# alexandre01/deepsvg

Measured on AMD Instinct MI355X. Metric: SVG icons/sec (train step) hierarchical_ordered d=256, higher is better.
Workload: dtype bf16; 1 GPU; hierarchical_ordered (Hierarchical, use_vae=False) G=8 S=30 d_model=256 ff=512 H=8 L=4x4; full train step = forward + SVGLoss + backward + grad-clip 1.0 + AdamW; dropout 0.1; global_batch=512, batch_per_gpu=512, parallelism=dp1, hip_graph=True, encoder_layout=packed (valid tokens only, exact)

## Files before the change

### deepsvg_amd/csrc/layernorm.hip

```cpp
#include "dsvg_common.h"
#include "../../include/dsvg.h"

constexpr int LN_MAXV_MAX = 4;
constexpr int LN_MAX_BLOCKS = 1024;

template <typename T, int LN_MAXV>
__global__ __launch_bounds__(256) void ln_fwd_kernel(const T* __restrict__ x, const float* __restrict__ gamma,
                                                     const float* __restrict__ beta, T* __restrict__ y,
                                                     float* __restrict__ mean, float* __restrict__ rstd,
                                                     long long rows, int d, float eps) {
    const int lane = threadIdx.x & 63;
    const int wave = threadIdx.x >> 6;
    const int nv = d / 256 + ((d % 256) ? 1 : 0);
    float4 g4[LN_MAXV], b4[LN_MAXV];
#pragma unroll
    for (int i = 0; i < LN_MAXV; ++i) {
        const int c = min(i * 256 + lane * 4, d - 4);
        g4[i] = *reinterpret_cast<const float4*>(gamma + c);
        b4[i] = *reinterpret_cast<const float4*>(beta + c);
    }
    for (long long row = (long long)blockIdx.x * 4 + wave; row < rows; row += (long long)gridDim.x * 4) {
        const T* xr = x + row * d;
        float v[LN_MAXV][4];
        float s = 0.f;
#pragma unroll
        for (int i = 0; i < LN_MAXV; ++i) {
            const int c = i * 256 + lane * 4;
            if (i < nv && c < d) {
                Elem<T>::ld4(xr + c, v[i]);
                s += v[i][0] + v[i][1] + v[i][2] + v[i][3];
            } else {
                v[i][0] = v[i][1] = v[i][2] = v[i][3] = 0.f;
            }
        }
        const float mu = wave_sum(s) / (float)d;
        float s2 = 0.f;
#pragma unroll
        for (int i = 0; i < LN_MAXV; ++i) {
            const int c = i * 256 + lane * 4;
            if (i < nv && c < d) {
#pragma unroll
                for (int e = 0; e < 4; ++e) { const float t = v[i][e] - mu; s2 += t * t; }
            }
        }
        const float var = wave_sum(s2) / (float)d;
        const float rs = rsqrtf(var + eps);
        if (lane == 0) { mean[row] = mu; rstd[row] = rs; }
        T* yr = y + row * d;
#pragma unroll
        for (int i = 0; i < LN_MAXV; ++i) {
            const int c = i * 256 + lane * 4;
            if (i < nv && c < d) {
                const float4 g = g4[i];
                const float4 b = b4[i];
                float o[4];
                o[0] = (v[i][0] - mu) * rs * g.x + b.x;
                o[1] = (v[i][1] - mu) * rs * g.y + b.y;
                o[2] = (v[i][2] - mu) * rs * g.z + b.z;
                o[3] = (v[i][3] - mu) * rs * g.w + b.w;
                Elem<T>::st4(yr + c, o);
            }
        }
    }
}

template <typename T, int LN_MAXV>
__global__ __launch_bounds__(256) void ln_bwd_kernel(const T* dy, const T* __restrict__ x,
                                                     const float* __restrict__ mean, const float* __restrict__ rstd,
                                                     const float* __restrict__ gamma, const T* res,
                                                     T* dx, float* __restrict__ part,
                                                     long long rows, int d, T* dxm, float drop_p,
                                                     const uint64_t* __restrict__ seed, uint32_t site) {
    const DropCtx dmc = drop_make(dxm ? drop_p : 0.f, seed, site);
    extern __shared__ float red_raw[];
    const int nvec = d / 4 + 1;
    auto red = [&](int w, int k, int vec, int e) -> float& { return red_raw[((w * 2 + k) * nvec + vec) * 4 + e]; };
    const int lane = threadIdx.x & 63;
    const int wave = threadIdx.x >> 6;
    const int nv = d / 256 + ((d % 256) ? 1 : 0);
    float ag[LN_MAXV][4], ab[LN_MAXV][4];
#pragma unroll
    for (int i = 0; i < LN_MAXV; ++i)
#pragma unroll
        for (int e = 0; e < 4; ++e) { ag[i][e] = 0.f; ab[i][e] = 0.f; }

    float4 g4[LN_MAXV];
#pragma unroll
    for (int i = 0; i < LN_MAXV; ++i) g4[i] = *reinterpret_cast<const float4*>(gamma + min(i * 256 + lane * 4, d - 4));
    for (long long row = (long long)blockIdx.x * 4 + wave; row < rows; row += (long long)gridDim.x * 4) {
        const float mu = mean[row], rs = rstd[row];
        float xh[LN_MAXV][4], gd[LN_MAXV][4], rv[LN_MAXV][4];
        float c1 = 0.f, c2 = 0.f;
#pragma unroll
        for (int i = 0; i < LN_MAXV; ++i) {
            const int c = i * 256 + lane * 4;
            if (i < nv && c < d) {
                float xv[4], dv[4];
                Elem<T>::ld4(x + row * d + c, xv);
                Elem<T>::ld4(dy + row * d + c, dv);
                if (res) Elem<T>::ld4(res + row * d + c, rv[i]);
                const float4 g = g4[i];
                const float gg[4] = {g.x, g.y, g.z, g.w};
#pragma unroll
                for (int e = 0; e < 4; ++e) {
                    xh[i][e] = (xv[e] - mu) * rs;
                    gd[i][e] = gg[e] * dv[e];
                    c1 += gd[i][e];
                    c2 += gd[i][e] * xh[i][e];
                    ag[i][e] += dv[e] * xh[i][e];
                    ab[i][e] += dv[e];
                }
            } else {
#pragma unroll
                for (int e = 0; e < 4; ++e) { xh[i][e] = 0.f; gd[i][e] = 0.f; }
// ... 83 lines not shown
    else if (dtype == DSVG_BF16) { if (d <= 256) DSVG_LNF(bf16_t, 1); else if (d <= 512) DSVG_LNF(bf16_t, 2); else DSVG_LNF(bf16_t, 4); }
    else { dsvg_set_error("layernorm_fwd: bad dtype %d", dtype); return -1; }
#undef DSVG_LNF
    DSVG_LAUNCH_CHECK("layernorm_fwd");
    return 0;
}

extern "C" int64_t dsvg_layernorm_bwd_workspace_bytes(int64_t rows, int32_t d) {
    return (int64_t)ln_grid(rows) * 2 * d * (int64_t)sizeof(float);
}

static int ln_bwd_launch(int32_t dtype, const void* dy, const void* x, const float* mean, const float* rstd,
                         const float* gamma, const void* res, void* dx, float* dgamma, float* dbeta,
                         int32_t accumulate, int64_t rows, int32_t d, float* workspace,
                         int64_t workspace_bytes, void* dx_masked, float drop_p, uint32_t drop_site, const void* seed,
                         void* stream);

extern "C" int dsvg_layernorm_bwd(int32_t dtype, const void* dy, const void* x, const float* mean, const float* rstd,
                                  const float* gamma, const void* res, void* dx, float* dgamma, float* dbeta,
                                  int32_t accumulate, int64_t rows, int32_t d, float* workspace,
                                  int64_t workspace_bytes, void* stream) {
    return ln_bwd_launch(dtype, dy, x, mean, rstd, gamma, res, dx, dgamma, dbeta, accumulate, rows, d, workspace,
                         workspace_bytes, nullptr, 0.f, 0u, nullptr, stream);
}

extern "C" int dsvg_layernorm_bwd_masked(int32_t dtype, const void* dy, const void* x, const float* mean, const float* rstd,
                                         const float* gamma, const void* res, void* dx, float* dgamma, float* dbeta,
                                         int32_t accumulate, int64_t rows, int32_t d, float* workspace,
                                         int64_t workspace_bytes, void* dx_masked, float drop_p, uint32_t drop_site,
                                         const void* seed, void* stream) {
    DSVG_CHECK_ARG(dx_masked && dx_masked != dx, "layernorm_bwd_masked: needs a second output buffer");
    DSVG_CHECK_ARG(!(drop_p > 0.f) || seed, "layernorm_bwd_masked: dropout needs a seed");
    return ln_bwd_launch(dtype, dy, x, mean, rstd, gamma, res, dx, dgamma, dbeta, accumulate, rows, d, workspace,
                         workspace_bytes, dx_masked, drop_p, drop_site, seed, stream);
}

static int ln_bwd_launch(int32_t dtype, const void* dy, const void* x, const float* mean, const float* rstd,
                         const float* gamma, const void* res, void* dx, float* dgamma, float* dbeta,
                         int32_t accumulate, int64_t rows, int32_t d, float* workspace,
                         int64_t workspace_bytes, void* dx_masked, float drop_p, uint32_t drop_site, const void* seed,
                         void* stream) {
    DSVG_CHECK_ARG(dy && x && mean && rstd && gamma && dx && dgamma && dbeta, "layernorm_bwd: null pointer");
    DSVG_CHECK_ARG(rows > 0 && d > 0 && (d % 4) == 0 && d <= 1024, "layernorm_bwd: bad shape");
    DSVG_CHECK_ARG(workspace && workspace_bytes >= dsvg_layernorm_bwd_workspace_bytes(rows, d),
                   "layernorm_bwd: workspace too small");
    hipStream_t st = (hipStream_t)stream;
    const int nb = ln_grid(rows);
    const size_t lds = (size_t)4 * 2 * (d / 4 + 1) * 4 * sizeof(float);
#define DSVG_LNB(TT, NV) hipLaunchKernelGGL((ln_bwd_kernel<TT, NV>), dim3(nb), dim3(256), lds, st, (const TT*)dy, \
                                            (const TT*)x, mean, rstd, gamma, (const TT*)res, (TT*)dx, workspace,  \
                                            (long long)rows, d, (TT*)dx_masked, drop_p, (const uint64_t*)seed, drop_site)
    if (dtype == DSVG_F32) { if (d <= 256) DSVG_LNB(float, 1); else if (d <= 512) DSVG_LNB(float, 2); else DSVG_LNB(float, 4); }
    else if (dtype == DSVG_BF16) { if (d <= 256) DSVG_LNB(bf16_t, 1); else if (d <= 512) DSVG_LNB(bf16_t, 2); else DSVG_LNB(bf16_t, 4); }
    else { dsvg_set_error("layernorm_bwd: bad dtype %d", dtype); return -1; }
#undef DSVG_LNB
    DSVG_LAUNCH_CHECK("layernorm_bwd");
    if (dbeta == dgamma + d)
        return dsvg_reduce_partials_strided(workspace, nb, 2 * (int64_t)d, 2 * (int64_t)d, dgamma, accumulate, st);
    int rc = 0;
    rc = dsvg_reduce_partials_strided(workspace, nb, 2 * (int64_t)d, d, dgamma, accumulate, st);
    if (rc) return rc;
    rc = dsvg_reduce_partials_strided(workspace + d, nb, 2 * (int64_t)d, d, dbeta, accumulate, st);
    return rc;
}
```

### deepsvg_amd/functional.py

```python
import math
import contextlib
import functools
import os

import torch

from . import ops

FFN_MIN_ROWS = int(os.environ.get("DSVG_FFN_MIN_ROWS", "16384"))
ATTN_MIN_ROWS = int(os.environ.get("DSVG_ATTN_MIN_ROWS", "16384"))
FFN_GATE_DW2 = os.environ.get("DSVG_FFN_GATE_DW2", "1") != "0"

LN_BWD_MASKED = os.environ.get("DSVG_LN_BWD_MASKED", "1") != "0"
DEFER_MORE = os.environ.get("DSVG_DEFER_MORE", "1") != "0"
HEAD_KPAD = os.environ.get("DSVG_HEAD_KPAD", "1") != "0"
GS_STACK = os.environ.get("DSVG_GS_STACK", "1") != "0"
_ATTN_VALU = os.environ.get("DSVG_ATTN_VALU") is not None
_ATTN_MFMA_MIN_S = int(os.environ.get("DSVG_ATTN_MFMA_MIN_S", "2"))
ATTN_BWD_DX = os.environ.get("DSVG_ATTN_BWD_DX", "0") != "0"
ATTN_BWD_DX_MIN_ROWS = int(os.environ.get("DSVG_ATTN_BWD_DX_MIN_ROWS", "8192"))
GS_REMAINDER = int(os.environ.get("DSVG_GS_REMAINDER", "512"))
SEQ_ROUND = 2048
HEAD_FUSED = os.environ.get("DSVG_HEAD_FUSED", "0") != "0"

# ... 271 lines not shown
            mk = (rt.p(ctx.mask_below[0]), ctx.mask_below[1], rt.seed)
        with rt.deferring():
            if live is None:
                out = ops.layernorm_bwd(dy, x, mean, rstd, gamma.detach(),
                                        dgamma=rt.grad_out(gamma), dbeta=rt.grad_out(beta), masked=mk)
                dx, dg, db = out[:3]
            else:
                R = live[1]
                dx = torch.empty_like(x)
                out = ops.layernorm_bwd(dy[:R], x[:R], mean[:R], rstd[:R], gamma.detach(), dx=dx[:R],
                                        dgamma=rt.grad_out(gamma), dbeta=rt.grad_out(beta), masked=mk)
                dg, db = out[1:3]
        if mk is not None:
            _hand_masked(rt, dx, out[3], mk[0], mk[1])
        return None, dx, dg, db, None, None, None


class AddPosFn(torch.autograd.Function):

    @staticmethod
    def forward(ctx, rt, x, pos_weight, n_seq, S, drop_rate, site, live=None):
        p = rt.p(drop_rate)
        y = ops.add_pos_fwd(x, pos_weight.detach(), n_seq, S, rt.dtype, p, site, rt.seed)
        ctx.rt, ctx.n_seq, ctx.S, ctx.p, ctx.site = rt, n_seq, S, p, site
        ctx.has_x = x is not None
        ctx.live = _live_rows(live, n_seq * S)
        assert ctx.live is None or x is None, "live-prefix backward is only wired for the constant embedding"
        ctx.save_for_backward(pos_weight)
        return y

# ... 766 lines not shown
```

### deepsvg_amd/lib.py

```python
import ctypes as C
import os

_HERE = os.path.dirname(os.path.abspath(__file__))
LIB_PATH = os.path.join(_HERE, "_lib", "libdsvg_hip.so")

DSVG_F32 = 0
DSVG_BF16 = 1
ABI_VERSION = 11

c_i32, c_i64, c_u32, c_f32 = C.c_int32, C.c_int64, C.c_uint32, C.c_float
vp = C.c_void_p


class GemmDesc(C.Structure):
    _fields_ = [
        ("dtype", c_i32), ("M", c_i32), ("N", c_i32), ("K", c_i32),
        ("A", vp), ("lda", c_i64), ("a_kc", c_i32),
        ("B", vp), ("ldb", c_i64), ("b_kc", c_i32),
        ("C", vp), ("ldc", c_i64), ("c_f32", c_i32),
        ("bias", vp),
        ("res", vp), ("ldres", c_i64), ("res_pre", c_i32),
        ("act", c_i32),
        ("gate", vp), ("ldgate", c_i64), ("gate_scale", c_f32),
        ("drop_p", c_f32), ("drop_site", c_u32),
# ... 23 lines not shown
    "dsvg_version": (c_i32, []),
    "dsvg_gemm": (c_i32, [C.POINTER(GemmDesc), vp]),
    "dsvg_gemm_workspace_bytes": (c_i64, [c_i32, c_i32, c_i32]),
    "dsvg_reduce_partials": (c_i32, [vp, c_i64, c_i64, vp, c_i32, vp]),
    "dsvg_defer_scope": (c_i32, [c_i32, vp]),
    "dsvg_flush_deferred": (c_i32, [vp]),
    "dsvg_defer_zero": (c_i32, [vp, c_i64, vp]),
    "dsvg_gemm_group_scope": (c_i32, [c_i32, vp]),
    "dsvg_colsum": (c_i32, [c_i32, vp, c_i64, c_i64, c_i32, vp, c_i32, c_f32, c_u32, vp, vp, c_i64, vp]),
    "dsvg_colsum_workspace_bytes": (c_i64, [c_i64, c_i32]),
    "dsvg_layernorm_fwd": (c_i32, [c_i32, vp, vp, vp, vp, vp, vp, c_i64, c_i32, c_f32, vp]),
    "dsvg_layernorm_bwd": (c_i32, [c_i32, vp, vp, vp, vp, vp, vp, vp, vp, vp, c_i32, c_i64, c_i32, vp, c_i64, vp]),
    "dsvg_layernorm_bwd_workspace_bytes": (c_i64, [c_i64, c_i32]),
    "dsvg_layernorm_bwd_masked": (c_i32, [c_i32, vp, vp, vp, vp, vp, vp, vp, vp, vp, c_i32, c_i64, c_i32, vp, c_i64, vp, c_f32,
                                          c_u32, vp, vp]),
    "dsvg_attention_fwd": (c_i32, [c_i32, vp, vp, vp, c_i64, vp, vp, c_i64, c_i32, c_i32, c_f32, c_f32, c_u32, vp, vp]),
    "dsvg_attention_bwd": (c_i32, [c_i32, vp, vp, vp, c_i64, vp, vp, vp, c_i64, c_i32, c_i32, c_f32, c_f32, c_u32, vp, vp]),
    "dsvg_attention_tiles": (c_i32, [vp, c_i64, c_i32, vp, vp, vp]),
    "dsvg_pack_tokens": (c_i32, [vp, vp, vp, c_i64, c_i32, c_i32, vp, vp, vp, vp, vp]),
    "dsvg_visible_first": (c_i32, [vp, c_i64, vp, vp, vp, vp]),
    "dsvg_head_pack_elems": (c_i64, [c_i32]),
    "dsvg_head_pack": (c_i32, [vp, c_i32, vp, vp]),
    "dsvg_head_argmax": (c_i32, [vp, vp, vp, c_i64, c_i32, c_i32, vp, vp]),
    "dsvg_head_sample": (c_i32, [vp, vp, vp, c_i64, c_i32, c_i32, c_f32, vp, c_u32, vp, vp]),
    "dsvg_head_lse_workspace_bytes": (c_i64, [c_i64]),
    "dsvg_head_lse": (c_i32, [vp, vp, vp, c_i64, c_i32, c_i32, vp, vp, vp, vp, vp, vp, c_i64, vp]),
    "dsvg_head_dlogits": (c_i32, [vp, vp, vp, c_i64, c_i32, c_i32, vp, vp, vp, vp, vp, vp, c_f32, vp, c_i64, vp]),
    "dsvg_attention_bwd_outproj": (c_i32, [vp, vp, vp, c_i64, vp, vp, vp, vp, c_i64, c_i32, c_f32, c_f32, c_u32, vp, vp]),
    "dsvg_attn_pack_bwd_elems": (c_i64, [c_i32]),
    "dsvg_attn_pack_bwd": (c_i32, [vp, vp, c_i32, vp, vp]),
# ... 122 lines not shown
```

### deepsvg_amd/model.py

```python
import math
import os

import torch
import torch.nn as nn

from . import ops
from . import functional as Fn
from .svgtensor import CMD_ARGS_MASK, EOS_ID, M_ID, SOS_ID

PACK_ONE_LAUNCH = os.environ.get("DSVG_PACK_ONE", "1") != "0"
PE_DROPOUT = 0.1


class ModelOutput(dict):
    _PENDING = object()

    def __init__(self, *a, **k):
        super().__init__(*a, **k)
        self._thunks = {}

    def set_lazy(self, key, fn):
        self._thunks[key] = fn
        dict.__setitem__(self, key, ModelOutput._PENDING)

# ... 563 lines not shown
    def seed_tensor(self, device):
        if self._seed is None or self._seed.device != device:
            self._seed = torch.tensor([torch.initial_seed() & 0x7FFFFFFFFFFFFFFF], dtype=torch.int64, device=device)
        return self._seed

    def _runtime(self, device):
        training = self.training
        seed = self.seed_tensor(device) if training else None
        self._store.ensure(device, self.compute_dtype, advance=(None, seed) if training and self._own_seed else None)
        self._rt = Fn.Runtime(self.compute_dtype, seed, self._store, training,
                              defer=self._defer_wgrad and (not ops.PROFILE_ON or ops.PROFILE_KEEP_DEFER))
        self._rt.path_stage = self.cfg.encode_stages == 2 or self.cfg.decode_stages == 2
        return self._rt

    def _run_stack(self, rt, stack, x, key_mask, z, n_seq, S, site, seq_off=None, live=None, tiles=None, l=None,
                   causal=False):
        cfg = self.cfg
        gl = None
        if z is not None and all(hasattr(L, "linear_global") for L in stack.layers) and self.hoist_global:
            wb = [t for L in stack.layers for t in (L.linear_global.weight, L.linear_global.bias)]
            gl = Fn.GlobalCondFn.apply(rt, z, *wb)
        n = len(stack.layers)
        all_g = all(hasattr(L, "linear_global") for L in stack.layers)
        if (n > 0 and not causal and seq_off is None and live is None and tiles is None and l is None
                and (z is None or (gl is not None and all_g))
                and Fn.gs_stack_eligible(rt, x, key_mask, n_seq, S, cfg.n_heads, n, [L.self_attn.in_proj_weight for L in stack.layers])):
            ts = []
            for i, L in enumerate(stack.layers):
                ts += [L.norm1.weight, L.norm1.bias, L.self_attn.in_proj_weight, L.self_attn.in_proj_bias,
                       L.self_attn.out_proj.weight, L.self_attn.out_proj.bias, L.norm2.weight, L.norm2.bias,
                       L.linear1.weight, L.linear1.bias, L.linear2.weight, L.linear2.bias]
                if z is not None:
                    ts.append(gl[i])
            x = Fn.GsStackFn.apply(rt, x, key_mask, n_seq, S, cfg.n_heads, cfg.dropout, site, n, z is not None, *ts)
            return Fn.LayerNormFn.apply(rt, x, stack.norm.weight, stack.norm.bias, stack.norm.eps, live, None)
        for i, L in enumerate(stack.layers):
            has_g = hasattr(L, "linear_global")
            has_l = l is not None and hasattr(L, "linear_global2")
            hoisted = gl is not None
            x = Fn.LayerFn.apply(
                rt, x, key_mask, (gl[i] if hoisted else z) if has_g else None, l if has_l else None, n_seq, S, cfg.n_heads,
                cfg.dropout, site + 8 * i,
                L.norm1.weight, L.norm1.bias, L.self_attn.in_proj_weight, L.self_attn.in_proj_bias,
                L.self_attn.out_proj.weight, L.self_attn.out_proj.bias, L.norm2.weight, L.norm2.bias,
                L.linear1.weight, L.linear1.bias, L.linear2.weight, L.linear2.bias,
                L.linear_global.weight if (has_g and not hoisted) else None,
                L.linear_global.bias if (has_g and not hoisted) else None,
                L.linear_global2.weight if has_l else None, L.linear_global2.bias if has_l else None,
                seq_off, live, tiles, causal,
                (site + 8 * (i - 1) + 4) if i > 0 else None, i == 0)
        n = len(stack.layers)
        return Fn.LayerNormFn.apply(rt, x, stack.norm.weight, stack.norm.bias, stack.norm.eps, live,
                                    (cfg.dropout, site + 8 * (n - 1) + 4) if (n > 0 and not rt.last_layer_gs) else None)

    def make_plan(self, commands_enc, args_enc, commands_dec, want_grad=True, args_dec=None):
        forced, self._forced_plan = self._forced_plan, None
        try:
            return self._plan(commands_enc, args_enc, commands_dec, want_grad, args_dec)
        finally:
            self._forced_plan = forced

    def _plan(self, commands_enc, args_enc, commands_dec, want_grad, args_dec=None):
        cfg = self.cfg
        if self._forced_plan is not None:
            return self._forced_plan
        plan = {"enc": None, "dec": None, "loss": None}
        ref = commands_enc if commands_enc is not None else commands_dec
        if ref is None or (ref.is_cuda and torch.cuda.is_current_stream_capturing()):
# ... 52 lines not shown
                    plan["loss"]["targets_r"] = (t[2].view(-1, n_args)[:, lo:hi].contiguous().view(-1),
                                                 t[3].view(-1, n_args)[:, lo:hi].contiguous().view(-1))
        return plan


    def _encode_stage1_packed(self, rt, pe, n_seq, S):
        enc = self.encoder
        emb = enc.embedding
        seq_off, pcmd, parg, ppos, total = pe["seq_off"], pe["pcmd"], pe["parg"], pe["ppos"], pe["total"]
        rows = min((total + 127) // 128 * 128, n_seq * S)
        rows = max(rows, min(int(pe.get("rows", 0)), n_seq * S))
        self.last_packing = (total, n_seq * S)
        src = Fn.PackedEmbedFn.apply(rt, pcmd[:rows], parg[:rows], ppos[:rows], S, PE_DROPOUT, 1,
                                     emb.command_embed.weight, emb.arg_embed.weight, emb.embed_fcn.weight,
                                     emb.embed_fcn.bias, emb.pos_encoding.pos_embed.weight)
        mem = self._run_stack(rt, enc.encoder, src, None, None, n_seq, S, 100, seq_off=seq_off, tiles=pe.get("tiles"))
        return Fn.MaskedMeanFn.apply(rt, mem, None, n_seq, S, seq_off)

    def _label_rows(self, rt, part, label, N):
        if label is None:
            raise ValueError("label_condition=True: forward needs `label`")
        label = label.reshape(-1)
        if label.numel() != N:
            raise ValueError(f"label has {label.numel()} entries for {N} icons")
        return Fn.LabelEmbedFn.apply(rt, label, part.label_embedding.label_embedding.weight)

    def _encode(self, rt, commands, args, plan=None, label=None):
        cfg = self.cfg
        enc = self.encoder
        N, G, S = commands.shape
        two = cfg.encode_stages == 2
        emb = enc.embedding
# ... 9 lines not shown
            cmd = commands.to(torch.float32).contiguous().view(N * G, S)
            arg = args.to(torch.float32).contiguous().view(N * G * S, -1)
            key_mask, _vis, group_mask = (ops.build_masks_lens if (two and S > 64) else ops.build_masks)(
                cmd, S, G, EOS_ID, want_group_mask=two)
            self.last_packing = None
            groups = ops.group_index(cmd, S, M_ID) if enc.use_group else None
            src = Fn.EmbedFn.apply(rt, cmd.view(-1), arg, groups, N * G, S, PE_DROPOUT, 1,
                                   emb.command_embed.weight, emb.arg_embed.weight, emb.embed_fcn.weight,
                                   emb.embed_fcn.bias, emb.pos_encoding.pos_embed.weight,
                                   emb.group_embed.weight if enc.use_group else None)
            mem = self._run_stack(rt, enc.encoder, src, key_mask, None, N * G, S, 100, l=l_seq)
            z = Fn.MaskedMeanFn.apply(rt, mem, key_mask, N * G, S)
        if two:
            src2 = z if cfg.self_match else \
                Fn.AddPosFn.apply(rt, z, enc.hierarchical_PE.pos_embed.weight, N, G, PE_DROPOUT, 2)
            mem2 = self._run_stack(rt, enc.hierarchical_encoder, src2, group_mask, None, N, G, 200, l=l)
            z = Fn.MaskedMeanFn.apply(rt, mem2, group_mask, N, G)
        return z

    def _bottleneck(self, rt, z):
        cfg = self.cfg
        mu = logsigma = None
        if (Fn.LATENT_FUSED and cfg.use_resnet and not cfg.use_vae and z.dtype == torch.bfloat16 and z.shape[1] == 256
                and tuple(self.bottleneck.bottleneck.weight.shape) == (256, 256) and rt.store is not None):
            wb = [t for i in range(1, 5) for t in (getattr(self.resnet, f"linear{i}")[0].weight,
                                                   getattr(self.resnet, f"linear{i}")[0].bias)]
            wb += [self.bottleneck.bottleneck.weight, self.bottleneck.bottleneck.bias]
            return Fn.LatentChainFn.apply(rt, z, *wb), mu, logsigma
        if cfg.use_resnet:
            for i in range(1, 5):
                lin = getattr(self.resnet, f"linear{i}")[0]
                z = Fn.ResBlockFn.apply(rt, z, lin.weight, lin.bias)
# ... 438 lines not shown
```

### deepsvg_amd/ops.py

```python
import ctypes as C
import os

import torch

from . import lib as _l

F32, BF16 = _l.DSVG_F32, _l.DSVG_BF16
RELU = 1

PROFILE_ON = False
PROFILE = []
PROFILE_KEEP_DEFER = False
_TAG = None


def _event():
    return torch.cuda.Event(enable_timing=True)


class tag:

    def __init__(self, name):
        self.name = name

# ... 373 lines not shown
        mp, msite, mseed = masked
        dxm = torch.empty_like(dx)
        _l.check(L.dsvg_layernorm_bwd_masked(_dt(x), dy.data_ptr(), x.data_ptr(), mean.data_ptr(), rstd.data_ptr(),
                                             gamma.data_ptr(), _p(res), dx.data_ptr(), dgamma.data_ptr(), dbeta.data_ptr(),
                                             int(accumulate), rows, d, ws.data_ptr(), ws.numel() * 4, dxm.data_ptr(),
                                             float(mp), int(msite), _p(mseed) if mp > 0 else None, _stream()),
                 "dsvg_layernorm_bwd_masked")
        _prof_end(ev, 0.0, 0.0, dict(op="layernorm_bwd"))
        return dx, dgamma, dbeta, dxm
    _l.check(L.dsvg_layernorm_bwd(_dt(x), dy.data_ptr(), x.data_ptr(), mean.data_ptr(), rstd.data_ptr(),
                                  gamma.data_ptr(), _p(res), dx.data_ptr(), dgamma.data_ptr(), dbeta.data_ptr(),
                                  int(accumulate), rows, d, ws.data_ptr(), ws.numel() * 4, _stream()),
             "dsvg_layernorm_bwd")
    _prof_end(ev, 0.0, 0.0, dict(op="layernorm_bwd"))
    return dx, dgamma, dbeta


def attention_tiles(seq_off, n_seq, max_rows=32):
    _chk(seq_off)
    assert seq_off.dtype == torch.int32 and seq_off.numel() == n_seq + 1
    tiles = torch.empty(n_seq + 2, dtype=torch.int32, device=seq_off.device)
    scratch = torch.empty((n_seq + 63) // 64 * 64, dtype=torch.int32, device=seq_off.device)
    _l.check(_l.load().dsvg_attention_tiles(seq_off.data_ptr(), n_seq, max_rows, tiles.data_ptr(), scratch.data_ptr(),
                                            _stream()), "dsvg_attention_tiles")
    return tiles


LONG_MFMA = os.environ.get("DSVG_LONG_MFMA", "1") != "0"


# ... 1237 lines not shown
```

### include/dsvg.h

```cpp
#ifndef DSVG_H
#define DSVG_H

#include <stdint.h>
#include <stddef.h>

#ifdef __cplusplus
extern "C" {
#endif

#define DSVG_F32 0
#define DSVG_BF16 1

#define DSVG_ABI_VERSION 11

const char* dsvg_last_error(void);
int dsvg_version(void);

typedef struct dsvg_gemm_desc {
    int32_t dtype;
    int32_t M, N, K;
    const void* A; int64_t lda; int32_t a_kc;
    const void* B; int64_t ldb; int32_t b_kc;
    void* C; int64_t ldc; int32_t c_f32;
    const float* bias;
    const void* res; int64_t ldres; int32_t res_pre;
    int32_t act;
    const void* gate; int64_t ldgate; float gate_scale;
    float drop_p; uint32_t drop_site;
// ... 20 lines not shown
                int32_t accumulate, float drop_p, uint32_t drop_site, const uint64_t* seed,
                float* workspace, int64_t workspace_bytes, void* stream);
int64_t dsvg_colsum_workspace_bytes(int64_t M, int32_t N);

int dsvg_layernorm_fwd(int32_t dtype, const void* x, const float* gamma, const float* beta, void* y,
                       float* mean, float* rstd, int64_t rows, int32_t d, float eps, void* stream);
int dsvg_layernorm_bwd(int32_t dtype, const void* dy, const void* x, const float* mean,
                       const float* rstd, const float* gamma, const void* res, void* dx,
                       float* dgamma, float* dbeta, int32_t accumulate, int64_t rows, int32_t d,
                       float* workspace, int64_t workspace_bytes, void* stream);
int64_t dsvg_layernorm_bwd_workspace_bytes(int64_t rows, int32_t d);
int dsvg_layernorm_bwd_masked(int32_t dtype, const void* dy, const void* x, const float* mean, const float* rstd,
                              const float* gamma, const void* res, void* dx, float* dgamma, float* dbeta,
                              int32_t accumulate, int64_t rows, int32_t d, float* workspace, int64_t workspace_bytes,
                              void* dx_masked, float drop_p, uint32_t drop_site, const void* seed, void* stream);

int dsvg_attention_fwd(int32_t dtype, const void* qkv, const uint64_t* key_mask, const int32_t* seq_off,
                       int64_t total_rows, const int32_t* tile_first, void* out, int64_t n_seq, int32_t S,
                       int32_t n_heads, float scale, float drop_p, uint32_t drop_site, const uint64_t* seed,
                       void* stream);
int dsvg_attention_bwd(int32_t dtype, const void* qkv, const uint64_t* key_mask, const int32_t* seq_off,
                       int64_t total_rows, const int32_t* tile_first, const void* dout, void* dqkv, int64_t n_seq,
                       int32_t S, int32_t n_heads, float scale, float drop_p, uint32_t drop_site,
                       const uint64_t* seed, void* stream);
int dsvg_attention_tiles(const int32_t* seq_off, int64_t n_seq, int32_t max_rows, int32_t* tile_first,
                         int32_t* scratch, void* stream);

int dsvg_build_masks(const float* commands, int64_t n_seq, int32_t S, int32_t G, int32_t eos_id,
                     uint64_t* key_mask, int32_t* seq_visible, uint64_t* group_mask, void* stream);

// ... 256 lines not shown
```

Before: 89430 icons/s.

## Fuse final encoder LayerNorm with masked mean pooling in forward and backward

Adds a fused kernel that runs the encoder's final LayerNorm and the masked mean pool over each sequence in one pass. It writes the pooled output plus a per-row map of sequence id and inverse count. Backward gets a LayerNorm variant that rebuilds the per-row gradient from the pooled gradient via that map, so the full-size normalized tensor and its gradient are never materialized. It is wired into both the packed first-level encoder and the hierarchical encoder. Bf16 rounding is emulated to keep results matching, and the path only handles d=256 with S≤64.

Result: no change. 89600 icons/s (median of 6 runs) (+0.2%).

```diff
diff --git a/deepsvg_amd/csrc/layernorm.hip b/deepsvg_amd/csrc/layernorm.hip
--- a/deepsvg_amd/csrc/layernorm.hip
+++ b/deepsvg_amd/csrc/layernorm.hip
@@ -1,4 +1,5 @@
 #include "dsvg_common.h"
+#include "ln_row.h"
 #include "../../include/dsvg.h"
 
 constexpr int LN_MAXV_MAX = 4;
@@ -22,55 +23,135 @@
     for (long long row = (long long)blockIdx.x * 4 + wave; row < rows; row += (long long)gridDim.x * 4) {
         const T* xr = x + row * d;
         float v[LN_MAXV][4];
-        float s = 0.f;
 #pragma unroll
         for (int i = 0; i < LN_MAXV; ++i) {
             const int c = i * 256 + lane * 4;
             if (i < nv && c < d) {
                 Elem<T>::ld4(xr + c, v[i]);
-                s += v[i][0] + v[i][1] + v[i][2] + v[i][3];
             } else {
                 v[i][0] = v[i][1] = v[i][2] = v[i][3] = 0.f;
             }
         }
-        const float mu = wave_sum(s) / (float)d;
-        float s2 = 0.f;
+        float mu, rs;
+        ln_row_stats<LN_MAXV>(v, nv, lane, d, eps, mu, rs);
+        if (lane == 0) { mean[row] = mu; rstd[row] = rs; }
+        T* yr = y + row * d;
 #pragma unroll
         for (int i = 0; i < LN_MAXV; ++i) {
             const int c = i * 256 + lane * 4;
             if (i < nv && c < d) {
-#pragma unroll
-                for (int e = 0; e < 4; ++e) { const float t = v[i][e] - mu; s2 += t * t; }
-            }
-        }
-        const float var = wave_sum(s2) / (float)d;
-        const float rs = rsqrtf(var + eps);
-        if (lane == 0) { mean[row] = mu; rstd[row] = rs; }
-        T* yr = y + row * d;
-#pragma unroll
-        for (int i = 0; i < LN_MAXV; ++i) {
-            const int c = i * 256 + lane * 4;
-            if (i < nv && c < d) {
-                const float4 g = g4[i];
-                const float4 b = b4[i];
                 float o[4];
-                o[0] = (v[i][0] - mu) * rs * g.x + b.x;
-                o[1] = (v[i][1] - mu) * rs * g.y + b.y;
-                o[2] = (v[i][2] - mu) * rs * g.z + b.z;
-                o[3] = (v[i][3] - mu) * rs * g.w + b.w;
+                ln_row_out4(v[i], mu, rs, g4[i], b4[i], o);
                 Elem<T>::st4(yr + c, o);
             }
         }
     }
 }
 
-template <typename T, int LN_MAXV>
+constexpr int LNM_ROWS = 8;
+__device__ __forceinline__ void lnm_load(const bf16_t* px, int i0, int last, uint2 (&t)[LNM_ROWS]) {
+#pragma unroll
+    for (int k = 0; k < LNM_ROWS; ++k) t[k] = *reinterpret_cast<const uint2*>(px + (long long)min(i0 + k, last) * 256);
+}
+__global__ __launch_bounds__(256) void ln_mean_fwd_kernel(const bf16_t* __restrict__ x, const float* __restrict__ gamma,
+                                                          const float* __restrict__ beta, const uint64_t* __restrict__ mask,
+                                                          const int32_t* __restrict__ seq_off, int S, bf16_t* __restrict__ out,
+                                                          float* __restrict__ mean, float* __restrict__ rstd,
+                                                          int2* __restrict__ row_map, long long n_seq, long long rows,
+                                                          float eps) {
+    constexpr int d = 256;
+    const int lane = threadIdx.x & 63;
+    const long long w = (long long)blockIdx.x * 4 + (threadIdx.x >> 6);
+    if (w >= n_seq) {
+        if (!seq_off) return;
+        const long long n_pad_waves = (long long)gridDim.x * 4 - n_seq;
+        for (long long row = (long long)seq_off[n_seq] + (w - n_seq); row < rows; row += n_pad_waves) {
+            if (row < 0) continue;
+            float v[1][4];
+            Elem<bf16_t>::ld4(x + row * d + lane * 4, v[0]);
+            float mu, rs;
+            ln_row_stats<1>(v, 1, lane, d, eps, mu, rs);
+            if (lane == 0) { mean[row] = mu; rstd[row] = rs; row_map[row] = make_int2(-1, 0); }
+        }
+        return;
+    }
+    const float4 g4 = *reinterpret_cast<const float4*>(gamma + lane * 4);
+    const float4 b4 = *reinterpret_cast<const float4*>(beta + lane * 4);
+    long long row0;
+    int len;
+    uint64_t m;
+    if (seq_off) {
+        row0 = seq_off[w];
+        len = seq_off[w + 1] - seq_off[w];
+        if (row0 < 0 || len < 0) len = 0;
+        if (len > 64) len = 64;
+        m = len >= 64 ? ~0ull : ((1ull << len) - 1ull);
+    } else {
+        row0 = w * S;
+        len = S;
+        m = mask[w];
+    }
+    if (row0 + len > rows) len = rows > row0 ? (int)(rows - row0) : 0;
+    const float inv = 1.f / (float)__popcll(m);
+    float acc[4] = {0.f, 0.f, 0.f, 0.f};
+    if (len > 0) {
+        const bf16_t* px = x + row0 * d + lane * 4;
+        uint2 cur[LNM_ROWS], nxt[LNM_ROWS];
+        lnm_load(px, 0, len - 1, cur);
+        float mu_l = 0.f, rs_l = 0.f;
+        for (int i0 = 0; i0 < len; i0 += LNM_ROWS) {
+            lnm_load(px, i0 + LNM_ROWS, len - 1, nxt);
+#pragma unroll
+            for (int k0 = 0; k0 < LNM_ROWS; k0 += 4) {
+                if (i0 + k0 < len) {
+                    float v[4][1][4], mu[4], rs[4];
+#pragma unroll
+                    for (int j = 0; j < 4; ++j) {
+                        const uint2 t = cur[k0 + j];
+                        v[j][0][0] = __uint_as_float(t.x << 16); v[j][0][1] = __uint_as_float(t.x & 0xffff0000u);
+                        v[j][0][2] = __uint_as_float(t.y << 16); v[j][0][3] = __uint_as_float(t.y & 0xffff0000u);
+                    }
+                    ln_rows_stats<4, 1>(v, 1, lane, d, eps, mu, rs);
+#pragma unroll
+                    for (int j = 0; j < 4; ++j) {
+                        const int k = k0 + j;
+                        if (lane == i0 + k) { mu_l = mu[j]; rs_l = rs[j]; }
+                        float o[4];
+                        ln_row_out4(v[j][0], mu[j], rs[j], g4, b4, o);
+                        bf16_t y[4];
+                        Elem<bf16_t>::st4(y, o);
+                        float yf[4];
+                        Elem<bf16_t>::ld4(y, yf);
+                        const bool counted = i0 + k < len && ((m >> ((i0 + k) & 63)) & 1ull);
+#pragma unroll
+                        for (int e = 0; e < 4; ++e) acc[e] = counted ? acc[e] + yf[e] : acc[e];
+                    }
+                }
+            }
+#pragma unroll
+            for (int k = 0; k < LNM_ROWS; ++k) cur[k] = nxt[k];
+        }
+        if (lane < len) {
+            const long long row = row0 + lane;
+            mean[row] = mu_l;
+            rstd[row] = rs_l;
+            const bool counted = (m >> lane) & 1ull;
+            row_map[row] = make_int2(counted ? (int)w : -1, __float_as_int(counted ? inv : 0.f));
+        }
+    }
+    const float o[4] = {acc[0] * inv, acc[1] * inv, acc[2] * inv, acc[3] * inv};
+    Elem<bf16_t>::st4(out + w * d + lane * 4, o);
+}
+
+template <typename T, int LN_MAXV, bool POOL = false>
 __global__ __launch_bounds__(256) void ln_bwd_kernel(const T* dy, const T* __restrict__ x,
                                                      const float* __restrict__ mean, const float* __restrict__ rstd,
                                                      const float* __restrict__ gamma, const T* res,
                                                      T* dx, float* __restrict__ part,
                                                      long long rows, int d, T* dxm, float drop_p,
-                                                     const uint64_t* __restrict__ seed, uint32_t site) {
+                                                     const uint64_t* __restrict__ seed, uint32_t site,
+                                                     const T* __restrict__ dpool = nullptr,
+                                                     const int2* __restrict__ row_map = nullptr, int n_seq = 0) {
     const DropCtx dmc = drop_make(dxm ? drop_p : 0.f, seed, site);
     extern __shared__ float red_raw[];
     const int nvec = d / 4 + 1;
@@ -87,8 +168,20 @@
     float4 g4[LN_MAXV];
 #pragma unroll
     for (int i = 0; i < LN_MAXV; ++i) g4[i] = *reinterpret_cast<const float4*>(gamma + min(i * 256 + lane * 4, d - 4));
+    int2 key_next = make_int2(-1, 0);
+    if constexpr (POOL) {
+        if ((long long)blockIdx.x * 4 + wave < rows) key_next = row_map[(long long)blockIdx.x * 4 + wave];
+    }
     for (long long row = (long long)blockIdx.x * 4 + wave; row < rows; row += (long long)gridDim.x * 4) {
         const float mu = mean[row], rs = rstd[row];
+        int b = -1;
+        float inv = 0.f;
+        if constexpr (POOL) {
+            const int2 key = key_next;
+            const long long nrow = row + (long long)gridDim.x * 4;
+            if (nrow < rows) key_next = row_map[nrow];
+            if ((unsigned)key.x < (unsigned)n_seq) { b = key.x; inv = __int_as_float(key.y); }
+        }
         float xh[LN_MAXV][4], gd[LN_MAXV][4], rv[LN_MAXV][4];
         float c1 = 0.f, c2 = 0.f;
 #pragma unroll
@@ -97,7 +190,20 @@
             if (i < nv && c < d) {
                 float xv[4], dv[4];
                 Elem<T>::ld4(x + row * d + c, xv);
-                Elem<T>::ld4(dy + row * d + c, dv);
+                if constexpr (POOL) {
+                    dv[0] = dv[1] = dv[2] = dv[3] = 0.f;
+                    if (b >= 0) {
+                        Elem<T>::ld4(dpool + (long long)b * d + c, dv);
+#pragma unroll
+                        for (int e = 0; e < 4; ++e) {
+                            T t;
+                            Elem<T>::st(&t, dv[e] * inv);
+                            dv[e] = Elem<T>::ld(&t);
+                        }
+                    }
+                } else {
+                    Elem<T>::ld4(dy + row * d + c, dv);
+                }
                 if (res) Elem<T>::ld4(res + row * d + c, rv[i]);
                 const float4 g = g4[i];
                 const float gg[4] = {g.x, g.y, g.z, g.w};
@@ -211,7 +317,7 @@
                          const float* gamma, const void* res, void* dx, float* dgamma, float* dbeta,
                          int32_t accumulate, int64_t rows, int32_t d, float* workspace,
                          int64_t workspace_bytes, void* dx_masked, float drop_p, uint32_t drop_site, const void* seed,
-                         void* stream);
+                         void* stream, const void* dpool = nullptr, const int32_t* row_map = nullptr, int64_t n_seq = 0);
 
 extern "C" int dsvg_layernorm_bwd(int32_t dtype, const void* dy, const void* x, const float* mean, const float* rstd,
                                   const float* gamma, const void* res, void* dx, float* dgamma, float* dbeta,
@@ -236,8 +342,8 @@
                          const float* gamma, const void* res, void* dx, float* dgamma, float* dbeta,
                          int32_t accumulate, int64_t rows, int32_t d, float* workspace,
                          int64_t workspace_bytes, void* dx_masked, float drop_p, uint32_t drop_site, const void* seed,
-                         void* stream) {
-    DSVG_CHECK_ARG(dy && x && mean && rstd && gamma && dx && dgamma && dbeta, "layernorm_bwd: null pointer");
+                         void* stream, const void* dpool, const int32_t* row_map, int64_t n_seq) {
+    DSVG_CHECK_ARG((dy || dpool) && x && mean && rstd && gamma && dx && dgamma && dbeta, "layernorm_bwd: null pointer");
     DSVG_CHECK_ARG(rows > 0 && d > 0 && (d % 4) == 0 && d <= 1024, "layernorm_bwd: bad shape");
     DSVG_CHECK_ARG(workspace && workspace_bytes >= dsvg_layernorm_bwd_workspace_bytes(rows, d),
                    "layernorm_bwd: workspace too small");
@@ -247,7 +353,11 @@
 #define DSVG_LNB(TT, NV) hipLaunchKernelGGL((ln_bwd_kernel<TT, NV>), dim3(nb), dim3(256), lds, st, (const TT*)dy, \
                                             (const TT*)x, mean, rstd, gamma, (const TT*)res, (TT*)dx, workspace,  \
                                             (long long)rows, d, (TT*)dx_masked, drop_p, (const uint64_t*)seed, drop_site)
-    if (dtype == DSVG_F32) { if (d <= 256) DSVG_LNB(float, 1); else if (d <= 512) DSVG_LNB(float, 2); else DSVG_LNB(float, 4); }
+    if (dpool)
+        hipLaunchKernelGGL((ln_bwd_kernel<bf16_t, 1, true>), dim3(nb), dim3(256), lds, st, (const bf16_t*)nullptr, (const bf16_t*)x,
+                           mean, rstd, gamma, (const bf16_t*)res, (bf16_t*)dx, workspace, (long long)rows, d, (bf16_t*)dx_masked,
+                           drop_p, (const uint64_t*)seed, drop_site, (const bf16_t*)dpool, (const int2*)row_map, (int)n_seq);
+    else if (dtype == DSVG_F32) { if (d <= 256) DSVG_LNB(float, 1); else if (d <= 512) DSVG_LNB(float, 2); else DSVG_LNB(float, 4); }
     else if (dtype == DSVG_BF16) { if (d <= 256) DSVG_LNB(bf16_t, 1); else if (d <= 512) DSVG_LNB(bf16_t, 2); else DSVG_LNB(bf16_t, 4); }
     else { dsvg_set_error("layernorm_bwd: bad dtype %d", dtype); return -1; }
 #undef DSVG_LNB
@@ -260,3 +370,32 @@
     rc = dsvg_reduce_partials_strided(workspace + d, nb, 2 * (int64_t)d, d, dbeta, accumulate, st);
     return rc;
 }
+
+extern "C" int dsvg_ln_mean_fwd(const void* x, const float* gamma, const float* beta, const uint64_t* mask,
+                                const int32_t* seq_off, void* out, float* mean, float* rstd, int32_t* row_map, int64_t n_seq,
+                                int32_t S, int64_t rows, int32_t d, float eps, void* stream) {
+    DSVG_CHECK_ARG(x && gamma && beta && out && mean && rstd && row_map, "ln_mean_fwd: null pointer");
+    DSVG_CHECK_ARG((mask != nullptr) != (seq_off != nullptr), "ln_mean_fwd: needs seq_off (packed) or mask (dense)");
+    DSVG_CHECK_ARG(n_seq > 0 && n_seq < (1ll << 31) && rows > 0 && S > 0 && S <= 64 && d == 256,
+                   "ln_mean_fwd: bad shape n_seq=%lld S=%d rows=%lld d=%d (d must be 256)", (long long)n_seq, S, (long long)rows, d);
+    DSVG_CHECK_ARG(seq_off || rows == n_seq * S, "ln_mean_fwd: dense layout has n_seq * S rows");
+    DSVG_CHECK_ARG((((uintptr_t)x | (uintptr_t)out | (uintptr_t)row_map) & 7) == 0 && (((uintptr_t)gamma | (uintptr_t)beta) & 15) == 0,
+                   "ln_mean_fwd: misaligned operand");
+    const long long nb = (n_seq + 3) / 4 + (seq_off ? 32 : 0);
+    hipLaunchKernelGGL(ln_mean_fwd_kernel, dim3((unsigned)nb), dim3(256), 0, (hipStream_t)stream, (const bf16_t*)x, gamma, beta,
+                       mask, seq_off, S, (bf16_t*)out, mean, rstd, (int2*)row_map, (long long)n_seq, (long long)rows, eps);
+    DSVG_LAUNCH_CHECK("ln_mean_fwd");
+    return 0;
+}
+
+extern "C" int dsvg_ln_mean_bwd(const void* dpool, const int32_t* row_map, int64_t n_seq, const void* x, const float* mean,
+                                const float* rstd, const float* gamma, void* dx, float* dgamma, float* dbeta,
+                                int32_t accumulate, int64_t rows, int32_t d, float* workspace, int64_t workspace_bytes,
+                                void* dx_masked, float drop_p, uint32_t drop_site, const void* seed, void* stream) {
+    DSVG_CHECK_ARG(dpool && row_map && ((uintptr_t)row_map & 7) == 0, "ln_mean_bwd: null or misaligned pointer");
+    DSVG_CHECK_ARG(d == 256 && n_seq > 0 && n_seq < (1ll << 31), "ln_mean_bwd: bad shape (d must be 256)");
+    DSVG_CHECK_ARG(dx_masked != dx, "ln_mean_bwd: the second output needs a buffer of its own");
+    DSVG_CHECK_ARG(!(dx_masked && drop_p > 0.f) || seed, "ln_mean_bwd: dropout needs a seed");
+    return ln_bwd_launch(DSVG_BF16, nullptr, x, mean, rstd, gamma, nullptr, dx, dgamma, dbeta, accumulate, rows, d, workspace,
+                         workspace_bytes, dx_masked, drop_p, drop_site, seed, stream, dpool, row_map, n_seq);
+}
diff --git a/deepsvg_amd/csrc/ln_row.h b/deepsvg_amd/csrc/ln_row.h
--- /dev/null
+++ b/deepsvg_amd/csrc/ln_row.h
@@ -0,0 +1,67 @@
+#pragma once
+#include "dsvg_common.h"
+
+template <int R>
+__device__ __forceinline__ void wave_sum_n(float (&s)[R]) {
+#pragma unroll
+    for (int o = 32; o > 0; o >>= 1) {
+        float t[R];
+#pragma unroll
+        for (int r = 0; r < R; ++r) t[r] = __shfl_xor(s[r], o, 64);
+        if constexpr (R == 4) asm volatile("" : "+v"(t[0]), "+v"(t[1]), "+v"(t[2]), "+v"(t[3]));
+#pragma unroll
+        for (int r = 0; r < R; ++r) s[r] += t[r];
+    }
+}
+
+template <int R, int NV>
+__device__ __forceinline__ void ln_rows_stats(const float (&v)[R][NV][4], int nv, int lane, int d, float eps, float (&mu)[R],
+                                              float (&rs)[R]) {
+#pragma clang fp contract(off)
+    float s[R];
+#pragma unroll
+    for (int r = 0; r < R; ++r) {
+        s[r] = 0.f;
+#pragma unroll
+        for (int i = 0; i < NV; ++i) {
+            const int c = i * 256 + lane * 4;
+            if (i < nv && c < d) s[r] += v[r][i][0] + v[r][i][1] + v[r][i][2] + v[r][i][3];
+        }
+    }
+    wave_sum_n<R>(s);
+    float s2[R];
+#pragma unroll
+    for (int r = 0; r < R; ++r) {
+        mu[r] = s[r] / (float)d;
+        s2[r] = 0.f;
+#pragma unroll
+        for (int i = 0; i < NV; ++i) {
+            const int c = i * 256 + lane * 4;
+            if (i < nv && c < d) {
+#pragma unroll
+                for (int e = 0; e < 4; ++e) { const float t = v[r][i][e] - mu[r]; s2[r] += t * t; }
+            }
+        }
+    }
+    wave_sum_n<R>(s2);
+#pragma unroll
+    for (int r = 0; r < R; ++r) {
+        const float var = s2[r] / (float)d;
+        rs[r] = rsqrtf(var + eps);
+    }
+}
+template <int NV>
+__device__ __forceinline__ void ln_row_stats(const float (&v)[NV][4], int nv, int lane, int d, float eps, float& mu, float& rs) {
+    float m1[1], r1[1];
+    ln_rows_stats<1, NV>(reinterpret_cast<const float (&)[1][NV][4]>(v), nv, lane, d, eps, m1, r1);
+    mu = m1[0];
+    rs = r1[0];
+}
+
+__device__ __forceinline__ void ln_row_out4(const float (&v)[4], float mu, float rs, const float4& g, const float4& b, float (&o)[4]) {
+#pragma clang fp contract(off)
+    o[0] = __builtin_fmaf((v[0] - mu) * rs, g.x, b.x);
+    o[1] = __builtin_fmaf((v[1] - mu) * rs, g.y, b.y);
+    o[2] = __builtin_fmaf((v[2] - mu) * rs, g.z, b.z);
+    o[3] = __builtin_fmaf((v[3] - mu) * rs, g.w, b.w);
+}
diff --git a/deepsvg_amd/functional.py b/deepsvg_amd/functional.py
--- a/deepsvg_amd/functional.py
+++ b/deepsvg_amd/functional.py
@@ -309,6 +309,40 @@
         if mk is not None:
             _hand_masked(rt, dx, out[3], mk[0], mk[1])
         return None, dx, dg, db, None, None, None
+
+
+GS_GLUE = os.environ.get("DSVG_GS_GLUE", "0") == "1"
+
+
+def ln_mean_eligible(x, mask, seq_off, S):
+    return (GS_GLUE and S <= 64 and x.is_cuda and x.dtype == torch.bfloat16 and x.dim() == 2 and x.shape[1] == 256
+            and (seq_off is not None or (mask is not None and mask.dtype == torch.int64)))
+
+
+class LnMeanFn(torch.autograd.Function):
+
+    @staticmethod
+    def forward(ctx, rt, x, gamma, beta, eps, mask, n_seq, S, seq_off=None, mask_below=None):
+        out, mean, rstd, row_map = ops.ln_mean_fwd(x, gamma.detach(), beta.detach(), eps, mask, n_seq, S, seq_off=seq_off)
+        ctx.rt = rt
+        ctx.mask_below = mask_below if (LN_BWD_MASKED and mask_below is not None and rt.p(mask_below[0]) > 0) else None
+        ctx.save_for_backward(x, mean, rstd, gamma, beta, row_map)
+        return out
+
+    @staticmethod
+    def backward(ctx, dout):
+        rt = ctx.rt
+        x, mean, rstd, gamma, beta, row_map = ctx.saved_tensors
+        mk = None
+        if ctx.mask_below is not None:
+            mk = (rt.p(ctx.mask_below[0]), ctx.mask_below[1], rt.seed)
+        with rt.deferring():
+            out = ops.ln_mean_bwd(dout.contiguous(), row_map, x, mean, rstd, gamma.detach(),
+                                  dgamma=rt.grad_out(gamma), dbeta=rt.grad_out(beta), masked=mk)
+        dx, dg, db = out[:3]
+        if mk is not None:
+            _hand_masked(rt, dx, out[3], mk[0], mk[1])
+        return None, dx, dg, db, None, None, None, None, None, None
 
 
 class AddPosFn(torch.autograd.Function):
diff --git a/deepsvg_amd/lib.py b/deepsvg_amd/lib.py
--- a/deepsvg_amd/lib.py
+++ b/deepsvg_amd/lib.py
@@ -6,7 +6,7 @@
 
 DSVG_F32 = 0
 DSVG_BF16 = 1
-ABI_VERSION = 11
+ABI_VERSION = 12
 
 c_i32, c_i64, c_u32, c_f32 = C.c_int32, C.c_int64, C.c_uint32, C.c_float
 vp = C.c_void_p
@@ -61,6 +61,9 @@
     "dsvg_layernorm_bwd_workspace_bytes": (c_i64, [c_i64, c_i32]),
     "dsvg_layernorm_bwd_masked": (c_i32, [c_i32, vp, vp, vp, vp, vp, vp, vp, vp, vp, c_i32, c_i64, c_i32, vp, c_i64, vp, c_f32,
                                           c_u32, vp, vp]),
+    "dsvg_ln_mean_fwd": (c_i32, [vp, vp, vp, vp, vp, vp, vp, vp, vp, c_i64, c_i32, c_i64, c_i32, c_f32, vp]),
+    "dsvg_ln_mean_bwd": (c_i32, [vp, vp, c_i64, vp, vp, vp, vp, vp, vp, vp, c_i32, c_i64, c_i32, vp, c_i64, vp, c_f32, c_u32, vp,
+                                 vp]),
     "dsvg_attention_fwd": (c_i32, [c_i32, vp, vp, vp, c_i64, vp, vp, c_i64, c_i32, c_i32, c_f32, c_f32, c_u32, vp, vp]),
     "dsvg_attention_bwd": (c_i32, [c_i32, vp, vp, vp, c_i64, vp, vp, vp, c_i64, c_i32, c_i32, c_f32, c_f32, c_u32, vp, vp]),
     "dsvg_attention_tiles": (c_i32, [vp, c_i64, c_i32, vp, vp, vp]),
diff --git a/deepsvg_amd/model.py b/deepsvg_amd/model.py
--- a/deepsvg_amd/model.py
+++ b/deepsvg_amd/model.py
@@ -601,7 +601,7 @@
         return self._rt
 
     def _run_stack(self, rt, stack, x, key_mask, z, n_seq, S, site, seq_off=None, live=None, tiles=None, l=None,
-                   causal=False):
+                   causal=False, pool=False):
         cfg = self.cfg
         gl = None
         if z is not None and all(hasattr(L, "linear_global") for L in stack.layers) and self.hoist_global:
@@ -620,7 +620,7 @@
                 if z is not None:
                     ts.append(gl[i])
             x = Fn.GsStackFn.apply(rt, x, key_mask, n_seq, S, cfg.n_heads, cfg.dropout, site, n, z is not None, *ts)
-            return Fn.LayerNormFn.apply(rt, x, stack.norm.weight, stack.norm.bias, stack.norm.eps, live, None)
+            return self._final_norm(rt, stack, x, key_mask, n_seq, S, None, None, None, pool)
         for i, L in enumerate(stack.layers):
             has_g = hasattr(L, "linear_global")
             has_l = l is not None and hasattr(L, "linear_global2")
@@ -637,8 +637,17 @@
                 seq_off, live, tiles, causal,
                 (site + 8 * (i - 1) + 4) if i > 0 else None, i == 0)
         n = len(stack.layers)
-        return Fn.LayerNormFn.apply(rt, x, stack.norm.weight, stack.norm.bias, stack.norm.eps, live,
-                                    (cfg.dropout, site + 8 * (n - 1) + 4) if (n > 0 and not rt.last_layer_gs) else None)
+        mask_below = (cfg.dropout, site + 8 * (n - 1) + 4) if (n > 0 and not rt.last_layer_gs) else None
+        return self._final_norm(rt, stack, x, key_mask, n_seq, S, seq_off, live, mask_below, pool)
+
+    @staticmethod
+    def _final_norm(rt, stack, x, key_mask, n_seq, S, seq_off, live, mask_below, pool):
+        norm = stack.norm
+        mask = key_mask if seq_off is None else None
+        if pool and live is None and Fn.ln_mean_eligible(x, mask, seq_off, S):
+            return Fn.LnMeanFn.apply(rt, x, norm.weight, norm.bias, norm.eps, mask, n_seq, S, seq_off, mask_below)
+        y = Fn.LayerNormFn.apply(rt, x, norm.weight, norm.bias, norm.eps, live, mask_below)
+        return Fn.MaskedMeanFn.apply(rt, y, mask, n_seq, S, seq_off) if pool else y
 
     def make_plan(self, commands_enc, args_enc, commands_dec, want_grad=True, args_dec=None):
         forced, self._forced_plan = self._forced_plan, None
@@ -721,8 +730,8 @@
         src = Fn.PackedEmbedFn.apply(rt, pcmd[:rows], parg[:rows], ppos[:rows], S, PE_DROPOUT, 1,
                                      emb.command_embed.weight, emb.arg_embed.weight, emb.embed_fcn.weight,
                                      emb.embed_fcn.bias, emb.pos_encoding.pos_embed.weight)
-        mem = self._run_stack(rt, enc.encoder, src, None, None, n_seq, S, 100, seq_off=seq_off, tiles=pe.get("tiles"))
-        return Fn.MaskedMeanFn.apply(rt, mem, None, n_seq, S, seq_off)
+        return self._run_stack(rt, enc.encoder, src, None, None, n_seq, S, 100, seq_off=seq_off, tiles=pe.get("tiles"),
+                               pool=True)
 
     def _label_rows(self, rt, part, label, N):
         if label is None:
@@ -762,8 +771,7 @@
         if two:
             src2 = z if cfg.self_match else \
                 Fn.AddPosFn.apply(rt, z, enc.hierarchical_PE.pos_embed.weight, N, G, PE_DROPOUT, 2)
-            mem2 = self._run_stack(rt, enc.hierarchical_encoder, src2, group_mask, None, N, G, 200, l=l)
-            z = Fn.MaskedMeanFn.apply(rt, mem2, group_mask, N, G)
+            z = self._run_stack(rt, enc.hierarchical_encoder, src2, group_mask, None, N, G, 200, l=l, pool=True)
         return z
 
     def _bottleneck(self, rt, z):
diff --git a/deepsvg_amd/ops.py b/deepsvg_amd/ops.py
--- a/deepsvg_amd/ops.py
+++ b/deepsvg_amd/ops.py
@@ -411,6 +411,51 @@
              "dsvg_layernorm_bwd")
     _prof_end(ev, 0.0, 0.0, dict(op="layernorm_bwd"))
     return dx, dgamma, dbeta
+
+
+def ln_mean_fwd(x, gamma, beta, eps, mask, n_seq, S, seq_off=None):
+    _chk(x, gamma, beta, mask, seq_off)
+    assert x.is_contiguous() and x.dim() == 2 and x.dtype == torch.bfloat16 and x.shape[1] == 256 and S <= 64
+    assert (mask is None) != (seq_off is None)
+    rows, d = x.shape
+    if seq_off is not None:
+        assert seq_off.dtype == torch.int32 and seq_off.numel() == n_seq + 1
+    else:
+        assert mask.dtype == torch.int64 and mask.numel() == n_seq and rows == n_seq * S
+    out = torch.empty((n_seq, d), dtype=x.dtype, device=x.device)
+    mean = torch.empty(rows, dtype=torch.float32, device=x.device)
+    rstd = torch.empty(rows, dtype=torch.float32, device=x.device)
+    row_map = torch.empty((rows, 2), dtype=torch.int32, device=x.device)
+    ev = _prof_begin()
+    _l.check(_l.load().dsvg_ln_mean_fwd(x.data_ptr(), gamma.data_ptr(), beta.data_ptr(), _p(mask), _p(seq_off), out.data_ptr(),
+                                        mean.data_ptr(), rstd.data_ptr(), row_map.data_ptr(), n_seq, S, rows, d, float(eps),
+                                        _stream()), "dsvg_ln_mean_fwd")
+    _prof_end(ev, 0.0, 0.0, dict(op="ln_mean_fwd"))
+    return out, mean, rstd, row_map
+
+
+def ln_mean_bwd(dpool, row_map, x, mean, rstd, gamma, *, dgamma=None, dbeta=None, accumulate=False, masked=None):
+    _chk(dpool, row_map, x, mean, rstd, gamma, dgamma, dbeta)
+    assert dpool.is_contiguous() and x.is_contiguous() and dpool.dtype == x.dtype == torch.bfloat16
+    rows, d = x.shape
+    assert d == 256 and dpool.dim() == 2 and dpool.shape[1] == d
+    assert row_map.dtype == torch.int32 and row_map.is_contiguous() and row_map.shape == (rows, 2)
+    dx = torch.empty_like(x)
+    if dgamma is None:
+        dgamma = torch.empty(d, dtype=torch.float32, device=x.device)
+    if dbeta is None:
+        dbeta = torch.empty(d, dtype=torch.float32, device=x.device)
+    L = _l.load()
+    ws = _ws(L.dsvg_layernorm_bwd_workspace_bytes(rows, d), x.device)
+    mp, msite, mseed = masked if masked is not None else (0.0, 0, None)
+    dxm = torch.empty_like(dx) if masked is not None else None
+    ev = _prof_begin()
+    _l.check(L.dsvg_ln_mean_bwd(dpool.data_ptr(), row_map.data_ptr(), dpool.shape[0], x.data_ptr(), mean.data_ptr(),
+                                rstd.data_ptr(), gamma.data_ptr(), dx.data_ptr(), dgamma.data_ptr(), dbeta.data_ptr(),
+                                int(accumulate), rows, d, ws.data_ptr(), ws.numel() * 4, _p(dxm), float(mp), int(msite),
+                                _p(mseed) if mp > 0 else None, _stream()), "dsvg_ln_mean_bwd")
+    _prof_end(ev, 0.0, 0.0, dict(op="ln_mean_bwd"))
+    return (dx, dgamma, dbeta) if masked is None else (dx, dgamma, dbeta, dxm)
 
 
 def attention_tiles(seq_off, n_seq, max_rows=32):
diff --git a/include/dsvg.h b/include/dsvg.h
--- a/include/dsvg.h
+++ b/include/dsvg.h
@@ -11,7 +11,7 @@
 #define DSVG_F32 0
 #define DSVG_BF16 1
 
-#define DSVG_ABI_VERSION 11
+#define DSVG_ABI_VERSION 12
 
 const char* dsvg_last_error(void);
 int dsvg_version(void);
@@ -62,6 +62,14 @@
                               const float* gamma, const void* res, void* dx, float* dgamma, float* dbeta,
                               int32_t accumulate, int64_t rows, int32_t d, float* workspace, int64_t workspace_bytes,
                               void* dx_masked, float drop_p, uint32_t drop_site, const void* seed, void* stream);
+
+int dsvg_ln_mean_fwd(const void* x, const float* gamma, const float* beta, const uint64_t* mask, const int32_t* seq_off,
+                     void* out, float* mean, float* rstd, int32_t* row_map, int64_t n_seq, int32_t S, int64_t rows, int32_t d,
+                     float eps, void* stream);
+int dsvg_ln_mean_bwd(const void* dpool, const int32_t* row_map, int64_t n_seq, const void* x, const float* mean,
+                     const float* rstd, const float* gamma, void* dx, float* dgamma, float* dbeta, int32_t accumulate,
+                     int64_t rows, int32_t d, float* workspace, int64_t workspace_bytes, void* dx_masked, float drop_p,
+                     uint32_t drop_site, const void* seed, void* stream);
 
 int dsvg_attention_fwd(int32_t dtype, const void* qkv, const uint64_t* key_mask, const int32_t* seq_off,
                        int64_t total_rows, const int32_t* tile_first, void* out, int64_t n_seq, int32_t S,
```
